# cgbur/llama2.zig

Hardware: AMD Instinct MI355X
Metric: tokens/s (argmax, -t 0) (higher is better)
Workload: dtype f32

## Files before the change

llama2.zig_amd/csrc/forward.cpp:

```cpp
#include <algorithm>
#include <cmath>
#include <cstdlib>
#include <cstring>
#include <mutex>

#include "l2z_state.h"

namespace l2z {

struct Prof {
    std::vector<hipEvent_t> ev;
    std::vector<int> kind;
};

#define L2Z_LAUNCH(kind_id, expr)                                                         \
    do {                                                                                  \
        hipEvent_t _a = nullptr, _b = nullptr;                                            \
        if (prof) {                                                                       \
            L2Z_HIP(hipEventCreate(&_a));                                                 \
            L2Z_HIP(hipEventCreate(&_b));                                                 \
            L2Z_HIP(hipEventRecord(_a, st));                                              \
        }                                                                                 \
        L2Z_HIP(expr);                                                                    \
        if (prof) {                                                                       \
// ... 94 lines not shown
        if (!can_push) return;
        a.push = s->d_push + which;
        a.push_ctl = ctl;
        a.push_gi = comm_gi(lc, gi + 1);
    };
    auto col_shard = [&](MatvecArgs &a, const float *wcols, const float *x_loc, int n_pad, int *epi) {
        a.w0 = wcols;
        a.x = x_loc;
        a.n = n_pad;
        a.rows0 = c.dim;
        a.out0 = s->part;
        a.resid = sh.rank == 0 ? s->x : nullptr;
        *epi = sh.rank == 0 ? EPI_RESID : EPI_STORE;
        push_to(a, 1);
    };
    for (int l = 0; l < c.n_layers; l++) {
        float *kc = s->key_cache + (size_t)l * c.seq_len * sh.kvd_loc;
        float *vc = s->value_cache + (size_t)l * c.seq_len * sh.kvd_loc;
        const size_t kvh_stride = (size_t)c.seq_len * sh.hs;
        const bool fused = s->fused_qkv_attn && !split && only_stage < 0;
        if (fused && kind(KIND_QKV)) {
            FusedQkvAttnArgs a = {};
            a.wq = w->wq + (size_t)l * dim * dim;
            a.wk = w->wk + (size_t)l * dim * dim;
            a.wv = w->wv + (size_t)l * dim * dim;
            a.rms_w = w->rms_att + (size_t)l * dim; a.x = s->x; a.q_out = s->q;
            a.kcache = kc; a.vcache = vc; a.xb = s->xb; a.pos_ptr = s->d_pos; a.rope = s->rope;
            a.n = c.dim; a.head_size = sh.hs; a.seq_len = c.seq_len; a.kv_dim = sh.kvd_loc;
            a.kv_row = sh.hs; a.kv_head = kvh_stride;
            L2Z_LAUNCH(KIND_QKV, launch_fused_qkv_attn(a, c.n_heads, st));
// ... 43 lines not shown
                push_to(a, 1);
            }
            L2Z_LAUNCH(KIND_WO, launch_matvec(a, PRO_NONE, epi, mb, g_cus, st, nullptr, &pushed));
        }
        if (sb) L2Z_TRY(reduce());
        else L2Z_TRY(gather(s->x, sh.dim_loc));
        if (want() && kind(KIND_FFN13)) {
            MatvecArgs a = {};
            a.w0 = w->w1 + (size_t)l * sh.hid_loc * 2 * dim;
            a.w1 = w->w3 + (size_t)l * sh.hid_loc * 2 * dim;
            a.out0 = sb ? s->hb : s->hb + sh.hid0;
            a.rows0 = sh.hid_loc; a.rows1 = sh.hid_loc; a.n = c.dim;
            a.rms_w = w->rms_ffn + (size_t)l * dim;
            x_in(a, s->x, gi, sh.dim_loc);
            if (!sb) push_to(a, 2);
            L2Z_LAUNCH(KIND_FFN13, launch_matvec(a, PRO_RMS, EPI_SWIGLU, mb, g_cus, st, nullptr, &pushed));
        }
        if (!sb) L2Z_TRY(gather(s->hb, sh.hid_loc));
        if (want() && kind(KIND_FFN2)) {
            MatvecArgs a = {};
            int epi = EPI_RESID;
            if (sb) {
                col_shard(a, w->w2 + (size_t)l * dim * sh.hidc_pad, s->hb, sh.hidc_pad, &epi);
            } else {
                a.w0 = w->w2 + (size_t)l * sh.dim_loc * hid;
                a.out0 = s->x + sh.dim0; a.resid = s->x + sh.dim0;
                a.rows0 = sh.dim_loc; a.n = c.hidden_dim;
                x_in(a, s->hb, gi, sh.hid_loc);
                push_to(a, 1);
            }
// ... 395 lines not shown
```

llama2.zig_amd/csrc/l2z_internal.h:

```cpp
#pragma once

#include <hip/hip_runtime.h>

#include <cstdarg>
#include <cstdint>
#include <cstdio>
#include <string>
#include <vector>

#include "../../include/llama2_hip.h"
#include "../../include/llama2_hip_test.h"

namespace l2z {

struct P2pArgs;

struct LLIn {
    const unsigned long long *slots;
    unsigned slot_floats;
    unsigned count;
    int gi;
    int *ctl;
    int *h_err;
    long long timeout_ticks;
// ... 65 lines not shown
    int n;
    const float *x;
    const float *rms_w;
    const float *resid;
    const int *pos_ptr;
    const float2 *rope;
    int head_size;
    int rope_segs;
    float *part_val;
    int *part_idx;
    int row_offset;
    const P2pArgs *push;
    const int *push_ctl;
    int push_gi;
    LLIn xin;
};

struct AttnArgs {
    const float *q;
    const float *kcache;
    const float *vcache;
    float *xb;
    const int *pos_ptr;
    int head_size;
    int kv_row;
    size_t kv_head;
    int kv_mul;
    int seq_len;
    const P2pArgs *push;
    const int *push_ctl;
// ... 6 lines not shown
    const float *wq, *wk, *wv;
    const float *rms_w, *x;
    float *q_out;
    float *kcache, *vcache;
    float *xb;
    const int *pos_ptr;
    const float2 *rope;
    int n;
    int head_size, seq_len, kv_dim;
    int kv_row;
    size_t kv_head;
};
bool fused_qkv_attn_supported(int dim, int n_heads, int n_kv_heads, int seq_len, int n_cus);
hipError_t launch_fused_qkv_attn(const FusedQkvAttnArgs &a, int n_heads, hipStream_t st);

hipError_t launch_matvec(const MatvecArgs &a, int pro, int epi, int max_blocks_per_cu, int n_cus,
                         hipStream_t st, int *out_grid = nullptr, bool *pushed = nullptr);
bool matvec_ll_supported(int n);
bool attention_push_supported(const AttnArgs &a);
int matvec_max_grid(int n_cus);
bool matvec_vector_width(int n);
hipError_t launch_stream_read(const float *p, size_t n_floats, float *out, int n_cus, hipStream_t st);
hipError_t launch_attention(const AttnArgs &a, int n_heads_local, hipStream_t st, int form = 0);
int attention_short_pos(int head_size, int seq_len);
int attention_split_chunks(int n_heads_local, int n_cus);
size_t attention_split_part_floats(int n_heads_local, int head_size, int nch);
bool attention_split_supported(const AttnArgs &a);
hipError_t launch_attention_split(const AttnArgs &a, int n_heads_local, int nch, float *part,
                                  int *arrivals, hipStream_t st, bool small = false);
int attention_split_wide_pos(int seq_len);
// ... 102 lines not shown
```

llama2.zig_amd/csrc/l2z_state.h:

```cpp
#pragma once
#include <cstdint>
#include <vector>

#include "l2z_comm.h"
#include "l2z_internal.h"
#include "tunables.h"

namespace l2z {

struct BatchScratch;

struct Shard {
    int rank = 0, world = 1;
    int hs = 0;
    int dim0 = 0, dim_loc = 0;
    int kvd_loc = 0;
    int heads_loc = 0;
    int hid0 = 0, hid_loc = 0;
    int v0 = 0, v_loc = 0;
    bool scheme_b = false;
    int dimc_pad = 0, hidc_pad = 0;
};
int pad_cols(int n);
int make_shard(const l2z_config &c, const l2z_comm *comm, Shard *out);
// ... 18 lines not shown
}

struct l2z_weights {
    uint64_t uid = 0;
    l2z_config cfg;
    int shared;
    int device;
    l2z::Shard sh;
    float *blob = nullptr;
    size_t blob_floats = 0;
    bool file_layout = false;
    std::vector<size_t> dev_off;
    const float *tok_emb = nullptr, *rms_att = nullptr, *rms_ffn = nullptr, *rms_final = nullptr;
    const float *wq = nullptr, *wk = nullptr, *wv = nullptr, *wo = nullptr;
    const float *w1 = nullptr, *w2 = nullptr, *w3 = nullptr, *wcls = nullptr;
};

enum { KIND_QKV = 0, KIND_ATTN, KIND_WO, KIND_FFN13, KIND_FFN2, KIND_CLS, KIND_ARGMAX, KIND_GATHER, KIND_COUNT };
static const char *const kKindNames[KIND_COUNT] = {"qkv", "attn", "wo", "ffn13", "ffn2", "cls", "argmax", "gather"};
static_assert(KIND_COUNT == L2Z_N_KINDS, "include/llama2_hip_test.h L2Z_N_KINDS");

struct l2z_runstate {
    l2z_config cfg;
    int device;
    l2z::Shard sh;
    const l2z_comm *comm = nullptr;
    hipStream_t stream = nullptr;
    float *x = nullptr, *xb = nullptr, *hb = nullptr, *q = nullptr, *logits = nullptr;
    float *part = nullptr;
    float *key_cache = nullptr, *value_cache = nullptr;
// ... 23 lines not shown
    int attn_short_pos = 0;
    int attn_split_wide_pos = 0;
    uint64_t graph_w_uid = 0;
    hipGraphExec_t g_forward[4] = {nullptr, nullptr, nullptr, nullptr}, g_step[4] = {nullptr, nullptr, nullptr, nullptr};
    bool use_graphs = true;
    int host_pos = 0;
    bool done = false;
    std::vector<int32_t> h_prompt;
    l2z::P2pArgs *d_push = nullptr;
    int n_gathers = 0;
    bool ll_consume = false;
    bool xchg_steps = false;
    bool logits_partial = false;
    bool fused_qkv_attn = false;
    int max_blocks = 0;
    int tl_attn_seq = 0;
    l2z::BatchScratch *bt = nullptr;
};

namespace l2z {

struct Prof;
int check_pair(const l2z_config *config, const l2z_runstate *s, const l2z_weights *w);
enum { ATTN_SHORT = 0, ATTN_HEAD = 1, ATTN_SPLIT_S = 2, ATTN_SPLIT = 3, ATTN_VARIANTS = 4 };
int enqueue_forward(l2z_runstate *s, const l2z_weights *w, bool with_step, Prof *prof, int only_stage,
                    int variant, int only_kind = -1);
int attn_variant(const l2z_runstate *s, int pos);
int run_forward(l2z_runstate *s, const l2z_weights *w, bool with_step, int pos);
int ensure_logits(l2z_runstate *s);
void drop_graphs(l2z_runstate *s);
// ... 12 lines not shown
```

llama2.zig_amd/csrc/matvec.hip:

```cpp
#include "matvec_device.h"

namespace l2z {
namespace {

__device__ __forceinline__ void dot2_scalar(const float *__restrict__ pa,
                                            const float *__restrict__ pb, const float *xs, int n,
                                            float &ra, float &rb)
{
    const int lane = threadIdx.x & 63;
    float sa = 0.0f, sb = 0.0f;
    for (int j = lane; j < n; j += kWave) {
        const float xv = xs[j];
        sa = fmaf(pa[j], xv, sa);
        sb = fmaf(pb[j], xv, sb);
    }
    ra = wave_sum(sa);
    rb = wave_sum(sb);
}

template <int LPR>
struct MvGeom {
    static constexpr int RW = kWave / LPR;
    static constexpr int U = (LPR == 64) ? 4 : 6;
};
// ... 132 lines not shown
            float bv = scratch[0];
            int bi = __float_as_int(scratch[kWaves]);
            for (int w = 1; w < kWaves; w++) {
                const float ov = scratch[w];
                const int oi = __float_as_int(scratch[kWaves + w]);
                if (oi != 0x7fffffff && (bi == 0x7fffffff || ov > bv || (ov == bv && oi < bi))) {
                    bv = ov; bi = oi;
                }
            }
            a.part_val[blockIdx.x] = bv;
            a.part_idx[blockIdx.x] = bi;
        }
    }
}

template <int PRO, int EPI, int XC, bool LL>
__global__ __launch_bounds__(kBlock) void matvec_row_kernel(const MatvecArgs a)
{
    constexpr int U = 4;
    extern __shared__ __attribute__((aligned(16))) float lds[];
    const MvLocals m = mv_locals<EPI>(a);
    const int n4 = m.n >> 2;
    const int n_batches = (n4 + kBlock * U - 1) / (kBlock * U);
    const int n4_pad = n_batches * (kBlock * U);
    float *xs = lds;
    float *scratch = lds + 4 * n4_pad;
    float *part = scratch + kScratch;
    const v4f *xs4 = (const v4f *)xs;
    const int tid = threadIdx.x, lane = tid & 63, wave = tid >> 6;
    const int n_units = m.n_pairs;
    const int ustride = gridDim.x;

    v4f xr[LL ? 1 : XC], gr[XC];
    v4u xl[LL ? 2 * XC : 2];
    LLPoll poll;
    if constexpr (LL) {
        poll = ll_poll_init(a.xin);
        xload_issue_ll<PRO, XC>(poll, a.rms_w, n4, xl, gr);
    } else {
        xload_issue<PRO, XC>(a.x, a.rms_w, n4, xr, gr);
    }
    int u = blockIdx.x;
    const float *pa, *pb;
    pair_rows<EPI>(m, u, pa, pb);
    v4f wa[U], wb[U];
    auto load = [&](int cb) {
        const v4f *a4 = (const v4f *)pa + cb + tid, *b4 = (const v4f *)pb + cb + tid;
        const int wbase = cb + (tid & ~63);
#pragma unroll
        for (int k = 0; k < U; k++) {
            const bool in_row = wbase + kBlock * k < n4;
            if (XC == 12 && !in_row) {
                wa[k] = v4f{0.f, 0.f, 0.f, 0.f};
                wb[k] = v4f{0.f, 0.f, 0.f, 0.f};
                continue;
            }
            const int off = in_row ? kBlock * k : -(cb + (tid & ~63));
            wa[k] = ldg_nt(a4 + off);
            wb[k] = ldg_nt(b4 + off);
        }
    };
    EpiIn ein = epi_prefetch<EPI>(m, u, tid == 0);
    EpiIn ein_next = ein;
    load(0);
    if constexpr (LL)
        xstage_finish_ll<PRO, XC>(poll, a.rms_w, m.n, n4_pad, xl, gr, xs, scratch);
    else
        xstage_finish<PRO, XC>(a.x, a.rms_w, m.n, n4_pad, xr, gr, xs, scratch);

    v4f acc_a = {0.f, 0.f, 0.f, 0.f}, acc_b = {0.f, 0.f, 0.f, 0.f};
    float best_v = -INFINITY;
    int best_i = 0x7fffffff;
    int b = 0, parity = 0;
    while (true) {
#pragma unroll
        for (int k = 0; k < U; k++) {
            const v4f xv = xs4[b * (kBlock * U) + tid + kBlock * k];
            acc_a = fma4(wa[k], xv, acc_a);
            acc_b = fma4(wb[k], xv, acc_b);
        }
        const bool unit_done = (b + 1 == n_batches);
        const int u_next = unit_done ? u + ustride : u;
        const int b_next = unit_done ? 0 : b + 1;
        const bool more = u_next < n_units;
        if (more) {
            if (unit_done) {
                pair_rows<EPI>(m, u_next, pa, pb);
                ein_next = epi_prefetch<EPI>(m, u_next, tid == 0);
            }
            load(b_next * (kBlock * U));
        }
        if (unit_done) {
            const float sa = wave_sum(hsum4(acc_a));
            const float sb = wave_sum(hsum4(acc_b));
            float *pp = part + parity * (2 * kWaves);
            if (lane == 0) {
                pp[wave] = sa;
                pp[kWaves + wave] = sb;
            }
            __syncthreads();
            if (tid == 0) {
                const float ta = ((pp[0] + pp[1]) + pp[2]) + pp[3];
                const float tb = ((pp[kWaves] + pp[kWaves + 1]) + pp[kWaves + 2]) + pp[kWaves + 3];
                pair_epilogue<EPI>(m, u, ta, tb, true, ein);
                if (EPI == EPI_ARGMAX) {
                    const int ra_ = 2 * u, rb_ = ra_ + 1;
                    if (ta > best_v || best_i == 0x7fffffff) { best_v = ta; best_i = ra_ + a.row_offset; }
                    if (rb_ < m.total_rows && tb > best_v) { best_v = tb; best_i = rb_ + a.row_offset; }
                }
            }
            ein = ein_next;
            parity ^= 1;
            acc_a = v4f{0.f, 0.f, 0.f, 0.f};
            acc_b = v4f{0.f, 0.f, 0.f, 0.f};
        }
        if (!more) break;
        u = u_next;
        b = b_next;
    }
    if (EPI == EPI_ARGMAX && tid == 0) {
        a.part_val[blockIdx.x] = best_v;
        a.part_idx[blockIdx.x] = best_i;
    }
}

template <int PRO, int EPI>
__global__ __launch_bounds__(kBlock) void matvec_scalar_kernel(const MatvecArgs a)
{
    extern __shared__ __attribute__((aligned(16))) float lds[];
    const MvLocals m = mv_locals<EPI>(a);
    float *xs = lds;
// ... 24 lines not shown
template <int PRO, int EPI, int LPR, int XC, bool LL>
MvLaunch mv_entry()
{
    return {reinterpret_cast<const void *>(&matvec_kernel<PRO, EPI, LPR, XC, LL>), LPR, MvGeom<LPR>::U};
}

template <int PRO, int EPI, bool LL>
MvLaunch mv_pick(int lpr, bool big_x)
{
    if (lpr == 8) return mv_entry<PRO, EPI, 8, 4, LL>();
    if (lpr == 16) return mv_entry<PRO, EPI, 16, 4, LL>();
    if (lpr == 32) return mv_entry<PRO, EPI, 32, 4, LL>();
    return big_x ? mv_entry<PRO, EPI, 64, 12, LL>() : mv_entry<PRO, EPI, 64, 4, LL>();
}

template <int PRO, int EPI, bool LL>
const void *mv_row_fn(bool big_x)
{
    return big_x ? reinterpret_cast<const void *>(&matvec_row_kernel<PRO, EPI, 12, LL>)
                 : reinterpret_cast<const void *>(&matvec_row_kernel<PRO, EPI, 4, LL>);
}

const void *mv_row_pick(int pro, int epi, bool big_x, bool ll)
{
#define L2Z_MVR(P, E) if (pro == P && epi == E && !ll) return mv_row_fn<P, E, false>(big_x);
#define L2Z_MVR_LL(P, E) if (pro == P && epi == E && ll) return mv_row_fn<P, E, true>(big_x);
    L2Z_MVR(PRO_NONE, EPI_STORE)
    L2Z_MVR(PRO_NONE, EPI_RESID)
    L2Z_MVR(PRO_RMS, EPI_STORE)
    L2Z_MVR(PRO_RMS, EPI_ROPE)
    L2Z_MVR(PRO_RMS, EPI_SWIGLU)
    L2Z_MVR(PRO_RMS, EPI_ARGMAX)
    L2Z_MVR_LL(PRO_NONE, EPI_RESID)
    L2Z_MVR_LL(PRO_RMS, EPI_STORE)
    L2Z_MVR_LL(PRO_RMS, EPI_ROPE)
// ... 70 lines not shown
    if (a.rows2 > 0) vec = vec && aligned16(a.w2);
    if (pro == PRO_RMS) vec = vec && aligned16(a.rms_w);
    if (epi == EPI_SWIGLU && a.rows1 != a.rows0) return hipErrorInvalidValue;
    const int total_rows = a.rows0 + a.rows1 + a.rows2;
    const int n_pairs = (epi == EPI_SWIGLU) ? a.rows0 : (total_rows + 1) / 2;
    if (n_pairs <= 0 || a.n <= 0) return hipErrorInvalidValue;
    const int n4 = a.n >> 2;
    const int lpr = lpr_for(n4);
    if (epi == EPI_ARGMAX && (!vec || a.rows1 != 0 || a.rows2 != 0)) return hipErrorNotSupported;
    const Tunables &tn = tunables();
    const bool use_row = vec && n4 >= 1024 && (n4 % 64) == 0;
    const bool ll = a.xin.slots != nullptr;
    if (ll && !vec) return hipErrorNotSupported;
    MvLaunch k = mv_pick_pe(pro, epi, lpr, a.n > 4096, vec, ll);
    if (use_row) k.fn = mv_row_pick(pro, epi, a.n > 4096, ll);
    if (k.fn == nullptr) return hipErrorInvalidValue;
    size_t lds;
    int n_units;
    if (use_row) {
        const int batch = kBlock * 4;
        const int n4_pad = ((n4 + batch - 1) / batch) * batch;
        lds = (size_t)(4 * n4_pad + kScratch + 4 * kWaves) * sizeof(float);
        n_units = n_pairs;
    } else if (vec) {
        const int batch = k.lpr * k.u;
        const int n4_pad = ((n4 + batch - 1) / batch) * batch;
        lds = (size_t)(4 * n4_pad + kScratch) * sizeof(float);
        const int rw = kWave / k.lpr;
        n_units = (n_pairs + rw - 1) / rw;
    } else {
// ... 38 lines not shown
```

llama2.zig_amd/csrc/matvec_device.h:

```cpp
#pragma once
#include "kernel_common.h"

namespace l2z {
namespace {

struct MvLocals {
    const float *w0, *w1, *w2;
    float *out0, *out1, *out2;
    const float *resid;
    const float2 *rope;
    int rows0, r01, total_rows, n_pairs, n, head_size, rope_segs, pos;
    size_t ps1, ps2;
    size_t kv_head_stride;
    const P2pArgs *push;
    int push_e;
    size_t push_base;
};

template <int EPI>
__device__ __forceinline__ MvLocals mv_locals(const MatvecArgs &a)
{
    MvLocals m;
    m.w0 = a.w0; m.w1 = a.w1; m.w2 = a.w2;
    m.out0 = a.out0; m.out1 = a.out1; m.out2 = a.out2;
    m.resid = a.resid; m.rope = a.rope;
    m.rows0 = a.rows0; m.r01 = a.rows0 + a.rows1; m.total_rows = a.rows0 + a.rows1 + a.rows2;
    m.n_pairs = (EPI == EPI_SWIGLU) ? a.rows0 : (m.total_rows + 1) >> 1;
    m.n = a.n; m.head_size = a.head_size; m.rope_segs = a.rope_segs;
    m.pos = (EPI == EPI_ROPE) ? *a.pos_ptr : 0;
    m.ps1 = (size_t)m.pos * (size_t)a.pos_stride1;
    m.ps2 = (size_t)m.pos * (size_t)a.pos_stride2;
    m.kv_head_stride = (EPI == EPI_ROPE) ? a.kv_head_stride : 0;
    m.push = a.push;
    m.push_e = m.push ? a.push_ctl[kCtlEpoch] + a.push_gi : 0;
    m.push_base = m.push ? (size_t)m.push->rank * m.push->count : 0;
    return m;
}

template <int EPI>
__device__ __forceinline__ void pair_rows(const MvLocals &m, int p, const float *&pa, const float *&pb)
{
    if (p >= m.n_pairs) p = m.n_pairs - 1;
    if (EPI == EPI_SWIGLU) {
        pa = m.w0 + (size_t)(2 * p) * (size_t)m.n;
        pb = pa + m.n;
    } else {
        const int ga = 2 * p;
        const int gb = (ga + 1 < m.total_rows) ? ga + 1 : ga;
        const bool a1 = ga >= m.rows0, a2 = ga >= m.r01;
        const bool b1 = gb >= m.rows0, b2 = gb >= m.r01;
        const int row_a = ga - (a2 ? m.r01 : (a1 ? m.rows0 : 0));
        const int row_b = gb - (b2 ? m.r01 : (b1 ? m.rows0 : 0));
        const float *wa = a1 ? m.w1 : m.w0;
        wa = a2 ? m.w2 : wa;
        const float *wb = b1 ? m.w1 : m.w0;
        wb = b2 ? m.w2 : wb;
        pa = wa + (size_t)row_a * (size_t)m.n;
        pb = wb + (size_t)row_b * (size_t)m.n;
    }
}

struct EpiIn {
    float ra, rb;
    float2 cs;
};

template <int EPI>
__device__ __forceinline__ EpiIn epi_prefetch(const MvLocals &m, int p, bool writer)
{
    EpiIn e;
    e.ra = 0.0f; e.rb = 0.0f; e.cs = make_float2(1.0f, 0.0f);
    if (!writer || p >= m.n_pairs) return e;
    if (EPI == EPI_RESID) {
        const int ga = 2 * p, gb = ga + 1;
// ... 82 lines not shown
```

llama2.zig_amd/csrc/runstate.cpp:

```cpp
#include <algorithm>
#include <cmath>
#include <cstdlib>
#include <cstring>
#include <mutex>
#include <vector>

#include "l2z_state.h"

using namespace l2z;

extern "C" int l2z_runstate_init(const l2z_config *config, const l2z_comm *comm, l2z_runstate **out)
{
    L2Z_CHECK(config != nullptr && out != nullptr, L2Z_ERR_INVALID, "runstate_init: null argument");
    const int dev = current_device_for(comm);
    L2Z_TRY(ensure_device(dev));
    Shard sh;
    L2Z_TRY(make_shard(*config, comm, &sh));
    const l2z_config &c = *config;
    const size_t att_lds = attention_lds_bytes(sh.hs, c.seq_len, sh.hs % 4 == 0 && sh.kvd_loc % 4 == 0);
    L2Z_CHECK(att_lds <= 160 * 1024, L2Z_ERR_INVALID,
              "seq_len %d needs %zu bytes of LDS for attention scores (max 163840)", c.seq_len,
              att_lds);
    const int n_max = c.dim > c.hidden_dim ? c.dim : c.hidden_dim;
    L2Z_CHECK(matvec_lds_bytes(n_max) <= 160 * 1024, L2Z_ERR_INVALID,
              "dim/hidden_dim %d does not fit the 160 KiB LDS x-staging buffer", n_max);

    l2z_runstate *s = new l2z_runstate();
    s->cfg = c;
    s->device = dev;
    s->sh = sh;
    s->comm = comm;
    const Tunables &tn = tunables();
    s->max_blocks = tn.max_blocks_per_cu;
    s->use_graphs = tn.no_graph == 0;
    if (comm && comm->world > 1 && !comm->nccl && !comm->p2p) s->use_graphs = false;
    s->fused_qkv_attn = sh.world == 1 && tn.fuse_small != 0 &&
                        fused_qkv_attn_supported(c.dim, c.n_heads, c.n_kv_heads, c.seq_len, g_cus);
    s->n_gathers = (sh.scheme_b ? 2 : 4) * c.n_layers + 1;
    if (comm_uses_p2p(comm)) {
        const size_t longest = std::max((size_t)std::max(std::max(c.dim, c.hidden_dim), c.vocab_size),
                                        sh.scheme_b ? (size_t)sh.world * (size_t)c.dim : (size_t)0);
        if (comm->slot_floats < longest) {
            set_error("peer-write landing slots hold %zu floats, this config gathers up to %zu: pass "
                      "max(dim, hidden_dim, vocab_size%s) to l2z_comm_p2p_export", comm->slot_floats, longest,
                      sh.scheme_b ? ", world * dim" : "");
            delete s;
            return L2Z_ERR_COMM;
        }
    }
// ... 241 lines not shown
```

llama2.zig_amd/csrc/tunables.cpp:

```cpp
#include "tunables.h"

#include <cstdlib>
#include <cstring>

namespace l2z {
namespace {

void env_int(const char *name, int *v)
{
    if (const char *e = getenv(name))
        if (*e) *v = atoi(e);
}

Tunables read_env()
{
    Tunables t;
    env_int("L2Z_GRID_CAP", &t.grid_cap);
    env_int("L2Z_ATTN_SPLIT", &t.attn_split);
    env_int("L2Z_ATTN_SPLIT_POS", &t.attn_split_pos);
    env_int("L2Z_FUSE_SMALL", &t.fuse_small);
    env_int("L2Z_SCHEME_B", &t.scheme_b);
    env_int("L2Z_NO_GRAPH", &t.no_graph);
    if (const char *e = getenv("L2Z_COMM")) t.prefer_rccl = strcmp(e, "rccl") == 0;
    env_int("L2Z_ARGMAX_XCHG", &t.argmax_xchg);
    env_int("L2Z_P2P_CONSUME", &t.p2p_consume);
    if (const char *e = getenv("L2Z_P2P_TIMEOUT_S"))
        if (*e) t.p2p_timeout_s = atoll(e);
    env_int("L2Z_P2P_BULK_MB", &t.p2p_bulk_mb);
    env_int("L2Z_PREFILL", &t.prefill);
    env_int("L2Z_PF_CHUNK", &t.pf_chunk);
    env_int("L2Z_PF_PANEL", &t.pf_panel);
    env_int("L2Z_PF_PANEL_MAX", &t.pf_panel_max);
    env_int("L2Z_PF_X3", &t.pf_x3);
    env_int("L2Z_PF_X3_STREAM_MIN", &t.pf_x3_stream_min);
    env_int("L2Z_PF_FUSE_PLANES", &t.pf_fuse_planes);
    return t;
}

}

namespace {
Tunables &mutable_tunables()
{
    static Tunables t = read_env();
    return t;
}
}

const Tunables &tunables() { return mutable_tunables(); }

// ... 9 lines not shown
{
    if (tunables().pf_chunk > 0) return remaining < prefill_chunk_tokens() ? remaining : prefill_chunk_tokens();
    return remaining >= 1024 ? 1024 : remaining < 512 ? remaining : 512;
}

bool tunables_set(const char *name, long long v)
{
    Tunables &t = mutable_tunables();
    struct { const char *n; int *p; } ints[] = {
        {"L2Z_GRID_CAP", &t.grid_cap}, {"L2Z_ATTN_SPLIT", &t.attn_split}, {"L2Z_ATTN_SPLIT_POS", &t.attn_split_pos},
        {"L2Z_FUSE_SMALL", &t.fuse_small}, {"L2Z_NO_GRAPH", &t.no_graph}, {"L2Z_SCHEME_B", &t.scheme_b},
        {"L2Z_COMM_RCCL", &t.prefer_rccl}, {"L2Z_ARGMAX_XCHG", &t.argmax_xchg}, {"L2Z_P2P_CONSUME", &t.p2p_consume},
        {"L2Z_P2P_BULK_MB", &t.p2p_bulk_mb}, {"L2Z_PREFILL", &t.prefill}, {"L2Z_PF_CHUNK", &t.pf_chunk},
        {"L2Z_PF_PANEL", &t.pf_panel}, {"L2Z_PF_PANEL_MAX", &t.pf_panel_max},
        {"L2Z_PF_X3", &t.pf_x3}, {"L2Z_PF_X3_STREAM_MIN", &t.pf_x3_stream_min},
        {"L2Z_PF_FUSE_PLANES", &t.pf_fuse_planes}};
    for (auto &e : ints)
        if (strcmp(e.n, name) == 0) {
            *e.p = (int)v;
            return true;
        }
    if (strcmp(name, "L2Z_P2P_TIMEOUT_S") == 0) {
        t.p2p_timeout_s = v;
        return true;
    }
    return false;
}

}
```

llama2.zig_amd/csrc/tunables.h:

```cpp
#pragma once

namespace l2z {

struct Tunables {
    int grid_cap = 0;
    int attn_split = -1;
    int attn_split_pos = -1;
    int fuse_small = 1;
    int no_graph = 0;
    int prefer_rccl = 0;
    int p2p_consume = -1;
    int argmax_xchg = 1;
    long long p2p_timeout_s = 20;
    int scheme_b = 0;
    int p2p_bulk_mb = -1;
    int prefill = 1;
    int pf_chunk = 0;
    int pf_panel = 1;
    int pf_x3 = 1;
    int pf_x3_stream_min = 33;
    int pf_fuse_planes = 1;
    int pf_panel_max = -1;

    static constexpr int row_blocks = 2;
    static constexpr int max_blocks_per_cu = 8;
    static constexpr int p2p_push = 1;
    static constexpr int reduce_block = 128;
    static constexpr int pf_skinny_max = 64;
};

const Tunables &tunables();
int prefill_chunk_tokens();
int prefill_next_chunk(int remaining);
bool tunables_set(const char *env_name, long long value);

}
// ... 1 lines not shown
```

llama2.zig_amd/csrc/weights.cpp:

```cpp
#include <algorithm>
#include <atomic>
#include <cmath>
#include <cstdlib>
#include <cstring>
#include <mutex>

#include "l2z_state.h"
#include "tunables.h"

namespace l2z {

static thread_local char g_err[512] = "";

void set_error(const char *fmt, ...)
{
    va_list ap;
    va_start(ap, fmt);
    vsnprintf(g_err, sizeof g_err, fmt, ap);
    va_end(ap);
}

int make_shard(const l2z_config &c, const l2z_comm *comm, Shard *out)
{
    Shard s;
// ... 201 lines not shown
    *tt_out = tensor_table(*config, w->shared != 0);
    w->blob_floats = local_floats(w, *tt_out);
    hipError_t e = hipMalloc(&w->blob, (w->blob_floats + kBlobSlackFloats) * sizeof(float));
    if (e == hipSuccess) e = hipMemset(w->blob + w->blob_floats, 0, kBlobSlackFloats * sizeof(float));
    if (e != hipSuccess) {
        set_error("hipMalloc(%zu bytes) for weights failed: %s", w->blob_floats * sizeof(float),
                  hipGetErrorString(e));
        delete w;
        return e == hipErrorOutOfMemory ? L2Z_ERR_OOM : L2Z_ERR_HIP;
    }
    carve_local(w, *tt_out);
    *out = w;
    return L2Z_OK;
}

}

extern "C" int l2z_abi_version(void) { return L2Z_ABI_VERSION; }
extern "C" const char *l2z_last_error(void) { return l2z::g_err; }

extern "C" int l2z_device_count(int *out_n)
{
    L2Z_CHECK(out_n != nullptr, L2Z_ERR_INVALID, "l2z_device_count: null out");
    int n = 0;
    hipError_t e = hipGetDeviceCount(&n);
    if (e != hipSuccess) n = 0;
    *out_n = n;
    return L2Z_OK;
}

// ... 52 lines not shown
            }
            if (e == hipSuccess) e = hipDeviceSynchronize();
        } else if (rl == d.rows) {
            e = upload(dst, data + d.offset, d.count());
        } else {
            for (size_t l = 0; l < d.layers && e == hipSuccess; l++)
                e = upload(dst + l * rl * d.cols, data + d.offset + (l * d.rows + r0) * d.cols, rl * d.cols);
        }
    }
    if (stage) (void)hipFree(stage);
    if (e != hipSuccess) {
        set_error("weight upload failed: %s", hipGetErrorString(e));
        l2z_weights_free(w);
        return L2Z_ERR_HIP;
    }
    *out = w;
    return L2Z_OK;
}

extern "C" int l2z_weights_init_synthetic(const l2z_config *config, int shared_weights,
                                          uint64_t seed, const l2z_comm *comm, l2z_weights **out)
{
    std::vector<TensorDesc> tt;
    l2z_weights *w = nullptr;
    L2Z_TRY(weights_alloc(config, shared_weights, comm, &w, &tt));
    hipError_t e = hipSuccess;
    for (size_t i = 0; i < tt.size(); i++) {
        const auto &d = tt[i];
        if (d.kind == SKIP && !w->file_layout) continue;
        size_t r0, r1;
// ... 9 lines not shown
                                      nullptr, cl, cpad, d.cols);
            continue;
        }
        for (size_t l = 0; l < d.layers && e == hipSuccess; l++) {
            const uint64_t base = d.offset + (l * d.rows + r0) * d.cols;
            e = launch_synth_fill(w->blob + w->dev_off[i] + l * rl * d.cols * (pair ? 2 : 1), base, rl * d.cols, seed, d.scale,
                                  d.bias, nullptr, pair ? d.cols : 0, pair ? 2 * d.cols : 0);
        }
    }
    if (e == hipSuccess) e = hipDeviceSynchronize();
    if (e != hipSuccess) {
        set_error("synthetic weight fill failed: %s", hipGetErrorString(e));
        l2z_weights_free(w);
        return L2Z_ERR_HIP;
    }
    *out = w;
    return L2Z_OK;
}

extern "C" int l2z_weights_read(const l2z_weights *w, size_t offset, size_t count, float *out)
{
    L2Z_CHECK(w != nullptr && out != nullptr, L2Z_ERR_INVALID, "l2z_weights_read: null argument");
    L2Z_CHECK(w->file_layout, L2Z_ERR_INVALID, "l2z_weights_read: only for unsharded weights");
    L2Z_CHECK(offset + count <= w->blob_floats, L2Z_ERR_INVALID, "l2z_weights_read: out of range");
    L2Z_HIP(hipSetDevice(w->device));
    const std::vector<TensorDesc> tt = tensor_table(w->cfg, w->shared != 0);
    const size_t lo = offset, hi = offset + count;
    for (size_t i = 0; i < tt.size(); i++) {
        const auto &d = tt[i];
        const size_t t0 = std::max(lo, d.offset), t1 = std::min(hi, d.offset + d.count());
// ... 13 lines not shown
                f += whole * d.cols;
            } else {
                const size_t n = std::min(d.cols - c, t1 - f);
                L2Z_HIP(hipMemcpy(out + (f - lo), src, n * sizeof(float), hipMemcpyDeviceToHost));
                f += n;
            }
        }
    }
    return L2Z_OK;
}

extern "C" void l2z_weights_free(l2z_weights *w)
{
    if (!w) return;
    if (w->blob) (void)hipFree(w->blob);
    delete w;
}
```

Before: 228.9.

## Pack FFN w1/w3 weights losslessly into 29-bit encoding to cut bandwidth

Adds a lossless 29-bit packing of the fused w1/w3 FFN weights: each layer's exponent range is measured, and if it spans at most 31 values the exponent is re-based into 5 bits and three spare bits per word carry extra values. A new packed variant of the row matvec kernel loads the packed stream, decodes it in registers and rescales with ldexp before the dot product, so about 9% fewer bytes are read for the largest matrix in decode. The cost is extra decode ALU work and register pressure in a bandwidth-bound kernel, plus a second copy of these weights in memory. It is enabled by default only for single-device, unsharded file-layout weights.

Result: faster. 236.7, median of 6 (+3.4%).

```diff
diff --git a/llama2.zig_amd/csrc/forward.cpp b/llama2.zig_amd/csrc/forward.cpp
--- a/llama2.zig_amd/csrc/forward.cpp
+++ b/llama2.zig_amd/csrc/forward.cpp
@@ -132,6 +132,7 @@
         *epi = sh.rank == 0 ? EPI_RESID : EPI_STORE;
         push_to(a, 1);
     };
+    const bool pk = s->packed_w && w->pk_blob != nullptr && !sb && sh.world == 1 && !consume;
     for (int l = 0; l < c.n_layers; l++) {
         float *kc = s->key_cache + (size_t)l * c.seq_len * sh.kvd_loc;
         float *vc = s->value_cache + (size_t)l * c.seq_len * sh.kvd_loc;
@@ -205,6 +206,7 @@
             a.rms_w = w->rms_ffn + (size_t)l * dim;
             x_in(a, s->x, gi, sh.dim_loc);
             if (!sb) push_to(a, 2);
+            if (pk && w->pk[l].p != nullptr) { a.pk = w->pk[l].p; a.pk_e = w->pk[l].e; }
             L2Z_LAUNCH(KIND_FFN13, launch_matvec(a, PRO_RMS, EPI_SWIGLU, mb, g_cus, st, nullptr, &pushed));
         }
         if (!sb) L2Z_TRY(gather(s->hb, sh.hid_loc));
diff --git a/llama2.zig_amd/csrc/l2z_internal.h b/llama2.zig_amd/csrc/l2z_internal.h
--- a/llama2.zig_amd/csrc/l2z_internal.h
+++ b/llama2.zig_amd/csrc/l2z_internal.h
@@ -103,6 +103,8 @@
     const int *push_ctl;
     int push_gi;
     LLIn xin;
+    const uint32_t *pk;
+    int pk_e;
 };
 
 struct AttnArgs {
@@ -139,6 +141,9 @@
 bool fused_qkv_attn_supported(int dim, int n_heads, int n_kv_heads, int seq_len, int n_cus);
 hipError_t launch_fused_qkv_attn(const FusedQkvAttnArgs &a, int n_heads, hipStream_t st);
 
+hipError_t launch_pk_stats(const float *m, size_t count, uint32_t *stats, hipStream_t st);
+hipError_t launch_pk_pack(const float *m, int rows, int n, int e_base, uint32_t *pk, hipStream_t st);
+hipError_t launch_pk_unpack(const uint32_t *pk, int rows, int n, int e_base, float *out, hipStream_t st);
 hipError_t launch_matvec(const MatvecArgs &a, int pro, int epi, int max_blocks_per_cu, int n_cus,
                          hipStream_t st, int *out_grid = nullptr, bool *pushed = nullptr);
 bool matvec_ll_supported(int n);
diff --git a/llama2.zig_amd/csrc/l2z_state.h b/llama2.zig_amd/csrc/l2z_state.h
--- a/llama2.zig_amd/csrc/l2z_state.h
+++ b/llama2.zig_amd/csrc/l2z_state.h
@@ -56,6 +56,13 @@
     const float *tok_emb = nullptr, *rms_att = nullptr, *rms_ffn = nullptr, *rms_final = nullptr;
     const float *wq = nullptr, *wk = nullptr, *wv = nullptr, *wo = nullptr;
     const float *w1 = nullptr, *w2 = nullptr, *w3 = nullptr, *wcls = nullptr;
+    struct PkMat {
+        const uint32_t *p = nullptr;
+        int e = 0;
+    };
+    uint32_t *pk_blob = nullptr;
+    std::vector<PkMat> pk;
+    int pk_packed = 0, pk_candidates = 0;
 };
 
 enum { KIND_QKV = 0, KIND_ATTN, KIND_WO, KIND_FFN13, KIND_FFN2, KIND_CLS, KIND_ARGMAX, KIND_GATHER, KIND_COUNT };
@@ -109,6 +116,7 @@
     bool logits_partial = false;
     bool fused_qkv_attn = false;
     int max_blocks = 0;
+    bool packed_w = true;
     int tl_attn_seq = 0;
     l2z::BatchScratch *bt = nullptr;
 };
diff --git a/llama2.zig_amd/csrc/matvec.hip b/llama2.zig_amd/csrc/matvec.hip
--- a/llama2.zig_amd/csrc/matvec.hip
+++ b/llama2.zig_amd/csrc/matvec.hip
@@ -1,4 +1,5 @@
 #include "matvec_device.h"
+#include "packed_w.h"
 
 namespace l2z {
 namespace {
@@ -170,7 +171,95 @@
     }
 }
 
-template <int PRO, int EPI, int XC, bool LL>
+struct PkRaw {
+    v4u q4[7];
+    uint32_t q1[3];
+};
+
+__device__ __forceinline__ void pk_load_raw(const uint32_t *src, int lane, int s, PkRaw &r)
+{
+    const int q = pk::lane_dw(s) / 4, rem = pk::lane_dw(s) % 4;
+#pragma unroll
+    for (int i = 0; i < 7; i++)
+        if (i < q) r.q4[i] = __builtin_nontemporal_load((const v4u *)(src + i * 256 + lane * 4));
+#pragma unroll
+    for (int i = 0; i < 3; i++)
+        if (i < rem) r.q1[i] = __builtin_nontemporal_load(src + q * 256 + i * 64 + lane);
+}
+
+template <int S>
+__device__ __forceinline__ void pk_decode_lane(const PkRaw &r, int e31, v4f (&wa)[4], v4f (&wb)[4])
+{
+    constexpr int N = pk::lane_dw(S), Q = N / 4;
+    uint32_t d[N > 0 ? N : 1], t[8 * S > 0 ? 8 * S : 1];
+#pragma unroll
+    for (int i = 0; i < N; i++) {
+        if (i < 4 * Q) {
+            const v4u v = r.q4[i / 4];
+            d[i] = (i % 4 == 0) ? v.x : (i % 4 == 1) ? v.y : (i % 4 == 2) ? v.z : v.w;
+        } else {
+            d[i] = r.q1[i - 4 * Q];
+        }
+    }
+    pk::decode_lane_t<S>(d, t);
+#pragma unroll
+    for (int k = 0; k < 4; k++) {
+        if (k < S) {
+            wa[k] = v4f{__builtin_amdgcn_ldexpf(__uint_as_float(t[8 * k]), e31), __builtin_amdgcn_ldexpf(__uint_as_float(t[8 * k + 1]), e31),
+                        __builtin_amdgcn_ldexpf(__uint_as_float(t[8 * k + 2]), e31), __builtin_amdgcn_ldexpf(__uint_as_float(t[8 * k + 3]), e31)};
+            wb[k] = v4f{__builtin_amdgcn_ldexpf(__uint_as_float(t[8 * k + 4]), e31), __builtin_amdgcn_ldexpf(__uint_as_float(t[8 * k + 5]), e31),
+                        __builtin_amdgcn_ldexpf(__uint_as_float(t[8 * k + 6]), e31), __builtin_amdgcn_ldexpf(__uint_as_float(t[8 * k + 7]), e31)};
+        } else {
+            wa[k] = v4f{0.f, 0.f, 0.f, 0.f};
+            wb[k] = v4f{0.f, 0.f, 0.f, 0.f};
+        }
+    }
+}
+
+typedef unsigned v2u_ __attribute__((ext_vector_type(2)));
+typedef unsigned v3u_ __attribute__((ext_vector_type(3)));
+
+template <int S>
+__device__ __forceinline__ void pk_load_lane(const uint32_t *src, int lane, uint32_t (&raw)[pk::kMaxLaneDw])
+{
+    constexpr int N = pk::lane_dw(S), Q = N / 4, R = N % 4;
+#pragma unroll
+    for (int q = 0; q < Q; q++) {
+        const v4u t = __builtin_nontemporal_load((const v4u *)(src + q * 256 + lane * 4));
+        raw[4 * q] = t.x; raw[4 * q + 1] = t.y; raw[4 * q + 2] = t.z; raw[4 * q + 3] = t.w;
+    }
+    const uint32_t *r = src + Q * 256 + lane * R;
+    if constexpr (R == 3) {
+        const v3u_ t = __builtin_nontemporal_load((const v3u_ *)r);
+        raw[4 * Q] = t.x; raw[4 * Q + 1] = t.y; raw[4 * Q + 2] = t.z;
+    } else if constexpr (R == 2) {
+        const v2u_ t = __builtin_nontemporal_load((const v2u_ *)r);
+        raw[4 * Q] = t.x; raw[4 * Q + 1] = t.y;
+    } else if constexpr (R == 1) {
+        raw[4 * Q] = __builtin_nontemporal_load(r);
+    }
+}
+
+template <int S>
+__device__ __forceinline__ void pk_decode_lane(const uint32_t (&raw)[pk::kMaxLaneDw], int e31, v4f (&wa)[4], v4f (&wb)[4])
+{
+    uint32_t t[8 * S > 0 ? 8 * S : 1];
+    pk::decode_lane_t<S>(raw, t);
+#pragma unroll
+    for (int k = 0; k < 4; k++) {
+        if (k < S) {
+            wa[k] = v4f{__builtin_amdgcn_ldexpf(__uint_as_float(t[8 * k]), e31), __builtin_amdgcn_ldexpf(__uint_as_float(t[8 * k + 1]), e31),
+                        __builtin_amdgcn_ldexpf(__uint_as_float(t[8 * k + 2]), e31), __builtin_amdgcn_ldexpf(__uint_as_float(t[8 * k + 3]), e31)};
+            wb[k] = v4f{__builtin_amdgcn_ldexpf(__uint_as_float(t[8 * k + 4]), e31), __builtin_amdgcn_ldexpf(__uint_as_float(t[8 * k + 5]), e31),
+                        __builtin_amdgcn_ldexpf(__uint_as_float(t[8 * k + 6]), e31), __builtin_amdgcn_ldexpf(__uint_as_float(t[8 * k + 7]), e31)};
+        } else {
+            wa[k] = v4f{0.f, 0.f, 0.f, 0.f};
+            wb[k] = v4f{0.f, 0.f, 0.f, 0.f};
+        }
+    }
+}
+
+template <int PRO, int EPI, int XC, bool LL, bool PK = false>
 __global__ __launch_bounds__(kBlock) void matvec_row_kernel(const MatvecArgs a)
 {
     constexpr int U = 4;
@@ -198,7 +287,7 @@
     }
     int u = blockIdx.x;
     const float *pa, *pb;
-    pair_rows<EPI>(m, u, pa, pb);
+    if constexpr (!PK) pair_rows<EPI>(m, u, pa, pb);
     v4f wa[U], wb[U];
     auto load = [&](int cb) {
         const v4f *a4 = (const v4f *)pa + cb + tid, *b4 = (const v4f *)pb + cb + tid;
@@ -216,9 +305,47 @@
             wb[k] = ldg_nt(b4 + off);
         }
     };
+    PkRaw raw, nraw;
+    int s_cur = 4, s_nxt = 4;
+    const int e31 = m.pk_e - 31;
+    const uint32_t *pp = nullptr;
+    size_t pdw = 0, last_off = 0;
+    int s_last = 4;
+    const int wave_u = __builtin_amdgcn_readfirstlane(wave);
+    auto pk_load = [&](int b_, PkRaw &dst, int &s_out) __attribute__((always_inline)) {
+        if constexpr (PK) {
+            const bool last = b_ + 1 == n_batches;
+            const uint32_t *src = pp + (last ? last_off : (size_t)b_ * (4 * 64 * pk::kMaxLaneDw) + (size_t)wave_u * (64 * pk::kMaxLaneDw));
+            s_out = (XC == 4 || !last) ? 4 : s_last;
+            pk_load_raw(src, lane, XC == 4 ? 4 : s_out, dst);
+        }
+    };
+    auto pk_decode = [&]() __attribute__((always_inline)) {
+        if constexpr (PK) {
+            if constexpr (XC == 4) {
+                pk_decode_lane<4>(raw, e31, wa, wb);
+            } else {
+                switch (s_cur) {
+                    case 4: pk_decode_lane<4>(raw, e31, wa, wb); break;
+                    case 3: pk_decode_lane<3>(raw, e31, wa, wb); break;
+                    case 2: pk_decode_lane<2>(raw, e31, wa, wb); break;
+                    case 1: pk_decode_lane<1>(raw, e31, wa, wb); break;
+                    default: pk_decode_lane<0>(raw, e31, wa, wb); break;
+                }
+            }
+        }
+    };
     EpiIn ein = epi_prefetch<EPI>(m, u, tid == 0);
     EpiIn ein_next = ein;
-    load(0);
+    if constexpr (PK) {
+        pdw = pk::pair_dw(n4);
+        last_off = pk::chunk_off(n4, n_batches - 1, wave_u);
+        s_last = pk::steps(n4, n_batches - 1, wave_u);
+        pp = pair_packed(m, u, pdw);
+        pk_load(0, raw, s_cur);
+    } else {
+        load(0);
+    }
     if constexpr (LL)
         xstage_finish_ll<PRO, XC>(poll, a.rms_w, m.n, n4_pad, xl, gr, xs, scratch);
     else
@@ -229,6 +356,19 @@
     int best_i = 0x7fffffff;
     int b = 0, parity = 0;
     while (true) {
+        if constexpr (PK) {
+            const bool unit_done = (b + 1 == n_batches);
+            const int u_next = unit_done ? u + ustride : u;
+            const int b_next = unit_done ? 0 : b + 1;
+            if (u_next < n_units) {
+                if (unit_done) {
+                    pp = pair_packed(m, u_next, pdw);
+                    ein_next = epi_prefetch<EPI>(m, u_next, tid == 0);
+                }
+                pk_load(b_next, nraw, s_nxt);
+            }
+            pk_decode();
+        }
 #pragma unroll
         for (int k = 0; k < U; k++) {
             const v4f xv = xs4[b * (kBlock * U) + tid + kBlock * k];
@@ -239,7 +379,7 @@
         const int u_next = unit_done ? u + ustride : u;
         const int b_next = unit_done ? 0 : b + 1;
         const bool more = u_next < n_units;
-        if (more) {
+        if (!PK && more) {
             if (unit_done) {
                 pair_rows<EPI>(m, u_next, pa, pb);
                 ein_next = epi_prefetch<EPI>(m, u_next, tid == 0);
@@ -249,15 +389,15 @@
         if (unit_done) {
             const float sa = wave_sum(hsum4(acc_a));
             const float sb = wave_sum(hsum4(acc_b));
-            float *pp = part + parity * (2 * kWaves);
+            float *pp_ = part + parity * (2 * kWaves);
             if (lane == 0) {
-                pp[wave] = sa;
-                pp[kWaves + wave] = sb;
+                pp_[wave] = sa;
+                pp_[kWaves + wave] = sb;
             }
             __syncthreads();
             if (tid == 0) {
-                const float ta = ((pp[0] + pp[1]) + pp[2]) + pp[3];
-                const float tb = ((pp[kWaves] + pp[kWaves + 1]) + pp[kWaves + 2]) + pp[kWaves + 3];
+                const float ta = ((pp_[0] + pp_[1]) + pp_[2]) + pp_[3];
+                const float tb = ((pp_[kWaves] + pp_[kWaves + 1]) + pp_[kWaves + 2]) + pp_[kWaves + 3];
                 pair_epilogue<EPI>(m, u, ta, tb, true, ein);
                 if (EPI == EPI_ARGMAX) {
                     const int ra_ = 2 * u, rb_ = ra_ + 1;
@@ -271,6 +411,10 @@
             acc_b = v4f{0.f, 0.f, 0.f, 0.f};
         }
         if (!more) break;
+        if constexpr (PK) {
+            raw = nraw;
+            s_cur = s_nxt;
+        }
         u = u_next;
         b = b_next;
     }
@@ -325,11 +469,17 @@
     return big_x ? mv_entry<PRO, EPI, 64, 12, LL>() : mv_entry<PRO, EPI, 64, 4, LL>();
 }
 
-template <int PRO, int EPI, bool LL>
+template <int PRO, int EPI, bool LL, bool PK = false>
 const void *mv_row_fn(bool big_x)
 {
-    return big_x ? reinterpret_cast<const void *>(&matvec_row_kernel<PRO, EPI, 12, LL>)
-                 : reinterpret_cast<const void *>(&matvec_row_kernel<PRO, EPI, 4, LL>);
+    return big_x ? reinterpret_cast<const void *>(&matvec_row_kernel<PRO, EPI, 12, LL, PK>)
+                 : reinterpret_cast<const void *>(&matvec_row_kernel<PRO, EPI, 4, LL, PK>);
+}
+
+const void *mv_row_pick_packed(int pro, int epi, bool big_x)
+{
+    if (pro == PRO_RMS && epi == EPI_SWIGLU) return mv_row_fn<PRO_RMS, EPI_SWIGLU, false, true>(big_x);
+    return nullptr;
 }
 
 const void *mv_row_pick(int pro, int epi, bool big_x, bool ll)
@@ -430,6 +580,10 @@
     if (ll && !vec) return hipErrorNotSupported;
     MvLaunch k = mv_pick_pe(pro, epi, lpr, a.n > 4096, vec, ll);
     if (use_row) k.fn = mv_row_pick(pro, epi, a.n > 4096, ll);
+    if (a.pk != nullptr) {
+        if (!use_row || ll || !pk::width_ok(a.n)) return hipErrorInvalidValue;
+        k.fn = mv_row_pick_packed(pro, epi, a.n > 4096);
+    }
     if (k.fn == nullptr) return hipErrorInvalidValue;
     size_t lds;
     int n_units;
diff --git a/llama2.zig_amd/csrc/matvec_device.h b/llama2.zig_amd/csrc/matvec_device.h
--- a/llama2.zig_amd/csrc/matvec_device.h
+++ b/llama2.zig_amd/csrc/matvec_device.h
@@ -15,6 +15,8 @@
     const P2pArgs *push;
     int push_e;
     size_t push_base;
+    const uint32_t *pk;
+    int pk_e;
 };
 
 template <int EPI>
@@ -34,6 +36,7 @@
     m.push = a.push;
     m.push_e = m.push ? a.push_ctl[kCtlEpoch] + a.push_gi : 0;
     m.push_base = m.push ? (size_t)m.push->rank * m.push->count : 0;
+    m.pk = a.pk; m.pk_e = a.pk_e;
     return m;
 }
 
@@ -58,6 +61,12 @@
         pa = wa + (size_t)row_a * (size_t)m.n;
         pb = wb + (size_t)row_b * (size_t)m.n;
     }
+}
+
+__device__ __forceinline__ const uint32_t *pair_packed(const MvLocals &m, int p, size_t pair_dw)
+{
+    if (p >= m.n_pairs) p = m.n_pairs - 1;
+    return m.pk + (size_t)p * pair_dw;
 }
 
 struct EpiIn {
diff --git a/llama2.zig_amd/csrc/packed_w.h b/llama2.zig_amd/csrc/packed_w.h
--- /dev/null
+++ b/llama2.zig_amd/csrc/packed_w.h
@@ -0,0 +1,95 @@
+#pragma once
+#include <cstddef>
+#include <cstdint>
+
+#ifndef __HIPCC__
+#define __host__
+#define __device__
+#endif
+
+namespace l2z {
+namespace pk {
+
+constexpr int kMaxLaneDw = 29;
+constexpr int kBatchF4 = 1024;
+
+__host__ __device__ constexpr int lane_dw(int s) { return (29 * s + 3) / 4; }
+__host__ __device__ constexpr int plane_off(int s, int i, int lane)
+{
+    return i < lane_dw(s) / 4 * 4 ? (i / 4) * 256 + lane * 4 + i % 4 : lane_dw(s) / 4 * 256 + (i - lane_dw(s) / 4 * 4) * 64 + lane;
+}
+
+__host__ __device__ inline int steps(int n4, int b, int w)
+{
+    int s = 0;
+    for (int k = 0; k < 4; k++) s += (b * kBatchF4 + 64 * w + 256 * k < n4) ? 1 : 0;
+    return s;
+}
+
+__host__ __device__ inline size_t chunk_off(int n4, int b, int w)
+{
+    size_t o = (size_t)b * 4 * 64 * kMaxLaneDw;
+    for (int v = 0; v < w; v++) o += (size_t)64 * lane_dw(steps(n4, b, v));
+    return o;
+}
+
+__host__ __device__ inline size_t pair_dw(int n4)
+{
+    const int nb = (n4 + kBatchF4 - 1) / kBatchF4;
+    return chunk_off(n4, nb - 1, 4);
+}
+
+__host__ __device__ constexpr bool width_ok(int n) { return n % 256 == 0 && n >= 4096; }
+
+__host__ __device__ inline uint32_t encode_t(uint32_t v, int e_base)
+{
+    const uint32_t e = (v >> 23) & 0xffu;
+    const uint32_t c = e == 0 ? 0u : e - (uint32_t)(e_base - 31);
+    return (v & 0x807fffffu) | (c << 23);
+}
+
+__host__ __device__ inline bool encodable(uint32_t max_e, uint32_t min_e, uint32_t bad)
+{
+    return bad == 0 && (max_e == 0 || min_e + 30 >= max_e);
+}
+
+template <int S>
+__host__ __device__ inline void encode_lane(const uint32_t *v, int e_base, uint32_t *d)
+{
+    constexpr int N = lane_dw(S), X = 8 * S - N;
+#pragma unroll
+    for (int i = 0; i < N; i++) d[i] = encode_t(v[i], e_base);
+#pragma unroll
+    for (int x = 0; x < X; x++) {
+        const uint32_t t = encode_t(v[N + x], e_base);
+        const uint32_t p = ((t << 1) | (t >> 31)) & 0x1fffffffu;
+#pragma unroll
+        for (int b = 0; b < 29; b++) {
+            const int s = 29 * x + b;
+            d[s / 3] |= ((p >> b) & 1u) << (28 + s % 3);
+        }
+    }
+}
+
+template <int S>
+__host__ __device__ inline void decode_lane_t(const uint32_t *d, uint32_t *t)
+{
+    constexpr int N = lane_dw(S), X = 8 * S - N;
+#pragma unroll
+    for (int i = 0; i < N; i++) t[i] = d[i] & 0x8fffffffu;
+#pragma unroll
+    for (int x = 0; x < X; x++) {
+        uint32_t p = 0;
+#pragma unroll
+        for (int q = (29 * x) / 3; q <= (29 * x + 28) / 3; q++) {
+            const int lo = 29 * x > 3 * q ? 29 * x : 3 * q;
+            const int hi = 29 * x + 29 < 3 * q + 3 ? 29 * x + 29 : 3 * q + 3;
+            const uint32_t piece = (d[q] >> (28 + lo - 3 * q)) & ((1u << (hi - lo)) - 1u);
+            p |= piece << (lo - 29 * x);
+        }
+        t[N + x] = (p >> 1) | (p << 31);
+    }
+}
+
+}
+}
diff --git a/llama2.zig_amd/csrc/packed_w.hip b/llama2.zig_amd/csrc/packed_w.hip
--- /dev/null
+++ b/llama2.zig_amd/csrc/packed_w.hip
@@ -0,0 +1,118 @@
+#include "kernel_common.h"
+#include "packed_w.h"
+
+namespace l2z {
+namespace {
+
+__global__ __launch_bounds__(256) void pk_stats_kernel(const uint32_t *__restrict__ p, size_t count, uint32_t *stats)
+{
+    uint32_t mx = 0, mn = 255, bad = 0;
+    for (size_t i = (size_t)blockIdx.x * 256 + threadIdx.x; i < count; i += (size_t)gridDim.x * 256) {
+        const uint32_t v = p[i], e = (v >> 23) & 0xffu;
+        if (e == 255u || (e == 0u && (v & 0x7fffffu) != 0u)) bad = 1;
+        if (e != 0u) {
+            mx = e > mx ? e : mx;
+            mn = e < mn ? e : mn;
+        }
+    }
+    for (int o = 32; o > 0; o >>= 1) {
+        const uint32_t omx = __shfl_xor(mx, o, 64), omn = __shfl_xor(mn, o, 64), ob = __shfl_xor(bad, o, 64);
+        mx = omx > mx ? omx : mx;
+        mn = omn < mn ? omn : mn;
+        bad |= ob;
+    }
+    if ((threadIdx.x & 63) == 0) {
+        atomicMax(stats + 0, mx);
+        atomicMin(stats + 1, mn);
+        if (bad) atomicOr(stats + 2, 1u);
+    }
+}
+
+template <int S>
+__device__ __forceinline__ void pk_pack_lane(const uint32_t *ra, const uint32_t *rb, int c4, int e_base, uint32_t *dst)
+{
+    uint32_t v[8 * S > 0 ? 8 * S : 1], d[pk::lane_dw(S) > 0 ? pk::lane_dw(S) : 1];
+#pragma unroll
+    for (int k = 0; k < S; k++)
+#pragma unroll
+        for (int j = 0; j < 4; j++) {
+            v[8 * k + j] = ra[4 * (c4 + 256 * k) + j];
+            v[8 * k + 4 + j] = rb[4 * (c4 + 256 * k) + j];
+        }
+#pragma unroll
+    for (int i = 0; i < pk::lane_dw(S); i++) d[i] = 0;
+    pk::encode_lane<S>(v, e_base, d);
+    const int lane = threadIdx.x & 63;
+#pragma unroll
+    for (int i = 0; i < pk::lane_dw(S); i++) dst[pk::plane_off(S, i, lane)] = d[i];
+}
+
+template <int S>
+__device__ __forceinline__ void pk_unpack_lane(const uint32_t *src, int c4, int e_base, uint32_t *oa, uint32_t *ob)
+{
+    const int lane = threadIdx.x & 63;
+    constexpr int N = pk::lane_dw(S);
+    uint32_t d[N > 0 ? N : 1], t[8 * S > 0 ? 8 * S : 1];
+#pragma unroll
+    for (int i = 0; i < N; i++) d[i] = src[pk::plane_off(S, i, lane)];
+    pk::decode_lane_t<S>(d, t);
+#pragma unroll
+    for (int k = 0; k < S; k++)
+#pragma unroll
+        for (int j = 0; j < 4; j++) {
+            oa[4 * (c4 + 256 * k) + j] = __float_as_uint(__builtin_amdgcn_ldexpf(__uint_as_float(t[8 * k + j]), e_base - 31));
+            ob[4 * (c4 + 256 * k) + j] = __float_as_uint(__builtin_amdgcn_ldexpf(__uint_as_float(t[8 * k + 4 + j]), e_base - 31));
+        }
+}
+
+template <bool PACK>
+__global__ __launch_bounds__(256) void pk_pack_kernel(const uint32_t *m, uint32_t *pk, uint32_t *out, int n, int e_base)
+{
+    const int n4 = n >> 2, q = blockIdx.x, b = blockIdx.y, w = threadIdx.x >> 6;
+    const int s = pk::steps(n4, b, w);
+    const size_t base = (size_t)q * pk::pair_dw(n4) + pk::chunk_off(n4, b, w);
+    const int c4 = b * pk::kBatchF4 + threadIdx.x;
+    const size_t ra = (size_t)(2 * q) * n, rb = ra + n;
+    switch (s) {
+#define L2Z_PK_CASE(S_)                                                            \
+    case S_:                                                                       \
+        if (PACK) pk_pack_lane<S_>(m + ra, m + rb, c4, e_base, pk + base);         \
+        else pk_unpack_lane<S_>(pk + base, c4, e_base, out + ra, out + rb);        \
+        break;
+        L2Z_PK_CASE(1)
+        L2Z_PK_CASE(2)
+        L2Z_PK_CASE(3)
+        L2Z_PK_CASE(4)
+#undef L2Z_PK_CASE
+        default: break;
+    }
+}
+
+}
+
+hipError_t launch_pk_stats(const float *m, size_t count, uint32_t *stats, hipStream_t st)
+{
+    size_t blocks = (count + 255) / 256;
+    if (blocks > 256 * 16) blocks = 256 * 16;
+    hipLaunchKernelGGL(pk_stats_kernel, dim3((unsigned)blocks), dim3(256), 0, st, (const uint32_t *)m, count, stats);
+    return hipGetLastError();
+}
+
+hipError_t launch_pk_pack(const float *m, int rows, int n, int e_base, uint32_t *pk, hipStream_t st)
+{
+    if (!pk::width_ok(n) || rows <= 0 || rows % 2) return hipErrorInvalidValue;
+    const dim3 grid(rows / 2, (n / 4 + pk::kBatchF4 - 1) / pk::kBatchF4);
+    hipLaunchKernelGGL(pk_pack_kernel<true>, grid, dim3(256), 0, st, (const uint32_t *)m, pk, nullptr, n, e_base);
+    return hipGetLastError();
+}
+
+hipError_t launch_pk_unpack(const uint32_t *pk, int rows, int n, int e_base, float *out, hipStream_t st)
+{
+    if (!pk::width_ok(n) || rows <= 0 || rows % 2) return hipErrorInvalidValue;
+    const dim3 grid(rows / 2, (n / 4 + pk::kBatchF4 - 1) / pk::kBatchF4);
+    hipLaunchKernelGGL(pk_pack_kernel<false>, grid, dim3(256), 0, st, nullptr, const_cast<uint32_t *>(pk),
+                       (uint32_t *)out, n, e_base);
+    return hipGetLastError();
+}
+
+}
diff --git a/llama2.zig_amd/csrc/runstate.cpp b/llama2.zig_amd/csrc/runstate.cpp
--- a/llama2.zig_amd/csrc/runstate.cpp
+++ b/llama2.zig_amd/csrc/runstate.cpp
@@ -33,6 +33,7 @@
     const Tunables &tn = tunables();
     s->max_blocks = tn.max_blocks_per_cu;
     s->use_graphs = tn.no_graph == 0;
+    s->packed_w = tn.packed_w != 0;
     if (comm && comm->world > 1 && !comm->nccl && !comm->p2p) s->use_graphs = false;
     s->fused_qkv_attn = sh.world == 1 && tn.fuse_small != 0 &&
                         fused_qkv_attn_supported(c.dim, c.n_heads, c.n_kv_heads, c.seq_len, g_cus);
diff --git a/llama2.zig_amd/csrc/tunables.cpp b/llama2.zig_amd/csrc/tunables.cpp
--- a/llama2.zig_amd/csrc/tunables.cpp
+++ b/llama2.zig_amd/csrc/tunables.cpp
@@ -34,6 +34,7 @@
     env_int("L2Z_PF_X3", &t.pf_x3);
     env_int("L2Z_PF_X3_STREAM_MIN", &t.pf_x3_stream_min);
     env_int("L2Z_PF_FUSE_PLANES", &t.pf_fuse_planes);
+    env_int("L2Z_PACKED_W", &t.packed_w);
     return t;
 }
 
@@ -73,7 +74,7 @@
         {"L2Z_P2P_BULK_MB", &t.p2p_bulk_mb}, {"L2Z_PREFILL", &t.prefill}, {"L2Z_PF_CHUNK", &t.pf_chunk},
         {"L2Z_PF_PANEL", &t.pf_panel}, {"L2Z_PF_PANEL_MAX", &t.pf_panel_max},
         {"L2Z_PF_X3", &t.pf_x3}, {"L2Z_PF_X3_STREAM_MIN", &t.pf_x3_stream_min},
-        {"L2Z_PF_FUSE_PLANES", &t.pf_fuse_planes}};
+        {"L2Z_PF_FUSE_PLANES", &t.pf_fuse_planes}, {"L2Z_PACKED_W", &t.packed_w}};
     for (auto &e : ints)
         if (strcmp(e.n, name) == 0) {
             *e.p = (int)v;
diff --git a/llama2.zig_amd/csrc/tunables.h b/llama2.zig_amd/csrc/tunables.h
--- a/llama2.zig_amd/csrc/tunables.h
+++ b/llama2.zig_amd/csrc/tunables.h
@@ -20,6 +20,7 @@
     int pf_x3 = 1;
     int pf_x3_stream_min = 33;
     int pf_fuse_planes = 1;
+    int packed_w = 1;
     int pf_panel_max = -1;
 
     static constexpr int row_blocks = 2;
diff --git a/llama2.zig_amd/csrc/weights.cpp b/llama2.zig_amd/csrc/weights.cpp
--- a/llama2.zig_amd/csrc/weights.cpp
+++ b/llama2.zig_amd/csrc/weights.cpp
@@ -6,6 +6,7 @@
 #include <mutex>
 
 #include "l2z_state.h"
+#include "packed_w.h"
 #include "tunables.h"
 
 namespace l2z {
@@ -239,6 +240,54 @@
     return L2Z_OK;
 }
 
+void build_packed(l2z_weights *w)
+{
+    if (tunables().packed_w == 0 || !w->file_layout) return;
+    const l2z_config &c = w->cfg;
+    const size_t dim = c.dim, hid = c.hidden_dim;
+    const int rows = 2 * c.hidden_dim, cols = c.dim, L = c.n_layers;
+    if (!pk::width_ok(cols)) return;
+    w->pk.assign(L, l2z_weights::PkMat{});
+    w->pk_candidates = L;
+    auto slot = [&](int l) { return w->w1 + (size_t)l * hid * 2 * dim; };
+    std::vector<uint32_t> stats(3 * (size_t)L);
+    for (int l = 0; l < L; l++) {
+        stats[3 * l] = 0;
+        stats[3 * l + 1] = 255;
+        stats[3 * l + 2] = 0;
+    }
+    uint32_t *d_stats = nullptr;
+    hipError_t e = hipMalloc((void **)&d_stats, stats.size() * sizeof(uint32_t));
+    if (e == hipSuccess) e = hipMemcpy(d_stats, stats.data(), stats.size() * sizeof(uint32_t), hipMemcpyHostToDevice);
+    for (int l = 0; l < L && e == hipSuccess; l++) e = launch_pk_stats(slot(l), (size_t)rows * cols, d_stats + 3 * l, nullptr);
+    if (e == hipSuccess) e = hipMemcpy(stats.data(), d_stats, stats.size() * sizeof(uint32_t), hipMemcpyDeviceToHost);
+    if (d_stats) (void)hipFree(d_stats);
+    const size_t per = (size_t)(rows / 2) * pk::pair_dw(cols / 4);
+    size_t total = 0;
+    for (int l = 0; l < L; l++) total += pk::encodable(stats[3 * l], stats[3 * l + 1], stats[3 * l + 2]) ? per : 0;
+    if (e == hipSuccess && total > 0) {
+        e = hipMalloc((void **)&w->pk_blob, total * sizeof(uint32_t));
+        if (e != hipSuccess) w->pk_blob = nullptr;
+    }
+    size_t off = 0;
+    for (int l = 0; l < L && e == hipSuccess && w->pk_blob; l++) {
+        if (!pk::encodable(stats[3 * l], stats[3 * l + 1], stats[3 * l + 2])) continue;
+        e = launch_pk_pack(slot(l), rows, cols, (int)stats[3 * l], w->pk_blob + off, nullptr);
+        w->pk[l].p = w->pk_blob + off;
+        w->pk[l].e = (int)stats[3 * l];
+        w->pk_packed++;
+        off += per;
+    }
+    if (e == hipSuccess) e = hipDeviceSynchronize();
+    if (e != hipSuccess) {
+        (void)hipGetLastError();
+        if (w->pk_blob) (void)hipFree(w->pk_blob);
+        w->pk_blob = nullptr;
+        w->pk.assign(L, l2z_weights::PkMat{});
+        w->pk_packed = 0;
+    }
+}
+
 }
 
 extern "C" int l2z_abi_version(void) { return L2Z_ABI_VERSION; }
@@ -321,6 +370,7 @@
         l2z_weights_free(w);
         return L2Z_ERR_HIP;
     }
+    build_packed(w);
     *out = w;
     return L2Z_OK;
 }
@@ -360,6 +410,7 @@
         l2z_weights_free(w);
         return L2Z_ERR_HIP;
     }
+    build_packed(w);
     *out = w;
     return L2Z_OK;
 }
@@ -403,5 +454,34 @@
 {
     if (!w) return;
     if (w->blob) (void)hipFree(w->blob);
+    if (w->pk_blob) (void)hipFree(w->pk_blob);
     delete w;
 }
+
+extern "C" int l2z_weights_packed_count(const l2z_weights *w, int *n_packed, int *n_candidates)
+{
+    L2Z_CHECK(w != nullptr && n_packed != nullptr && n_candidates != nullptr, L2Z_ERR_INVALID,
+              "l2z_weights_packed_count: null argument");
+    *n_packed = w->pk_packed;
+    *n_candidates = w->pk_candidates;
+    return L2Z_OK;
+}
+
+extern "C" int l2z_weights_packed_read(const l2z_weights *w, int layer, float *out, size_t n_floats)
+{
+    L2Z_CHECK(w != nullptr && out != nullptr, L2Z_ERR_INVALID, "l2z_weights_packed_read: null argument");
+    L2Z_CHECK(layer >= 0 && (size_t)layer < w->pk.size(), L2Z_ERR_INVALID, "l2z_weights_packed_read: no packed layer %d", layer);
+    const auto &pm = w->pk[layer];
+    L2Z_CHECK(pm.p != nullptr, L2Z_ERR_STATE, "l2z_weights_packed_read: layer %d is not packed", layer);
+    const int rows = 2 * w->cfg.hidden_dim, cols = w->cfg.dim;
+    const size_t count = (size_t)rows * cols;
+    L2Z_CHECK(n_floats >= count, L2Z_ERR_INVALID, "l2z_weights_packed_read: need %zu floats", count);
+    L2Z_HIP(hipSetDevice(w->device));
+    float *d = nullptr;
+    L2Z_HIP(hipMalloc((void **)&d, count * sizeof(float)));
+    hipError_t e = launch_pk_unpack(pm.p, rows, cols, pm.e, d, nullptr);
+    if (e == hipSuccess) e = hipMemcpy(out, d, count * sizeof(float), hipMemcpyDeviceToHost);
+    (void)hipFree(d);
+    L2Z_HIP(e);
+    return L2Z_OK;
+}
```
